# baycom/tfrec

Measured on AMD Instinct MI355X. Metric: IQ MSamples/s through demod+decode (batched streams), higher is better.
Workload: dtype int32+f32+f64

## Files before the change

tfrec_amd/csrc/decode.h:

```cpp
#pragma once

__device__ __forceinline__ const uint32_t *win_bits(const WinTables &T, int c, int j, int og)
{
	return T.bits + (size_t)c * T.bit_words + (og >> 6) + 3 * j;
}

__device__ __forceinline__ uint32_t tfa1_sr_before(const WinTables &T, const ChainState &st, int c, int j)
{
	uint32_t sr = 0;
	int have = 0;
	for (int k = j - 1; k >= 0 && have < 32; k--) {
		const int nb = T.result[(size_t)c * T.cap + k].nbits;
		if (nb <= 0)
			continue;
		const uint32_t *bits = win_bits(T, c, k, T.open[(size_t)c * T.cap + k]);
		const int take = nb < 32 - have ? nb : 32 - have;
		const int p0 = nb - take;
		const uint32_t lo = bits[p0 >> 5], hi = ((p0 + take - 1) >> 5) != (p0 >> 5) ? bits[(p0 >> 5) + 1] : 0u;
		const unsigned long long w = ((unsigned long long)hi << 32) | lo;
		const uint32_t piece = (uint32_t)(w >> (p0 & 31)) & (take >= 32 ? ~0u : (1u << take) - 1u);
		sr = (have == 0) ? (take >= 32 ? piece : piece << (32 - take))
				 : (sr | (piece << (32 - have - take)));
		have += take;
	}
	if (have < 32)
		sr |= have ? (st.sr >> have) : st.sr;
	return sr;
}

template <int KIND>
__device__ __forceinline__ void decode_window(int c, int j, int n_streams, const ChainLaunch &L, const WinTables &T,
					      uint8_t *__restrict__ my_rdata)
{
	const int a = c / n_streams, s = c - a * n_streams;
	const ChainState &st = L.states[a][s];
	const WinResult r = T.result[(size_t)c * T.cap + j];
	const int og = T.open[(size_t)c * T.cap + j];
	const uint32_t *bits = win_bits(T, c, j, og);
	Dec d{ 0u, -1, 0, 0, 0, 0, 0, 0, 0, 0u, 0u, my_rdata };
	if (j == 0) {
		const uint4 *src = reinterpret_cast<const uint4 *>(st.rdata);
		uint4 *dst = reinterpret_cast<uint4 *>(my_rdata);
#pragma unroll
		for (int q = 0; q < 4; q++)
			dst[q] = src[q];
		d.sr = st.sr;
		d.sr_cnt = st.sr_cnt;
		d.byte_cnt = st.byte_cnt;
		d.invert = st.invert;
	} else if (KIND == 0) {
		d.sr = tfa1_sr_before(T, st, c, j);
	}
	int maxlen = d.byte_cnt;
	const int nbits = r.nbits;
	uint32_t wnext = nbits > 0 ? bits[0] : 0u;
	for (int n = 0; n < nbits; n += 32) {
		const uint32_t wbits = wnext;
		if (n + 32 < nbits)
			wnext = bits[(n >> 5) + 1];
		const int cnt = nbits - n < 32 ? nbits - n : 32;
		for (int q = 0; q < cnt; q++) {
			store_bit<KIND>(d, (wbits >> q) & 1);
			maxlen = d.byte_cnt > maxlen ? d.byte_cnt : maxlen;
		}
	}
	WinDecode &o = T.decode[(size_t)c * T.cap + j];
	o.sr = d.sr;
	o.sr_cnt = d.sr_cnt;
	o.byte_cnt = d.byte_cnt;
	o.invert = d.invert;
	o.wlen = j == 0 ? 64 : (maxlen < 64 ? maxlen : 64);
	const uint4 *src = reinterpret_cast<const uint4 *>(my_rdata);
	uint4 *dst = reinterpret_cast<uint4 *>(o.vals);
#pragma unroll
	for (int q = 0; q < 4; q++)
		dst[q] = src[q];
}

__global__ __launch_bounds__(64) void decode_kernel(int n_streams, ChainLaunch L, WinTables T, int kind)
{
	__builtin_amdgcn_s_setprio(3);
	__shared__ __attribute__((aligned(16))) uint8_t rdata_lds[64 * 256];
	uint8_t *my_rdata = rdata_lds + 256 * threadIdx.x;
	const size_t total = (size_t)L.n_active * n_streams * T.cap;
	const uint32_t tid = blockIdx.x * 64 + threadIdx.x, nthreads = gridDim.x * 64;
	for (int q = 2 * kind; q < 2 * kind + 2; q++) {
		const uint32_t count = T.queue[q].count;
		for (uint32_t idx = tid; idx < count; idx += nthreads) {
			const uint2 it = T.items[(size_t)q * total + idx];
			if (kind == 0)
				decode_window<0>((int)it.x, (int)it.y, n_streams, L, T, my_rdata);
			else
				decode_window<1>((int)it.x, (int)it.y, n_streams, L, T, my_rdata);
		}
	}
}

template <int KIND, bool WAVE>
__device__ __forceinline__ void commit_body(int a, int s, int n_streams, int n_blocks, long long sample_base,
					    const uint32_t *__restrict__ dec, size_t dec_stride,
					    const int16_t *__restrict__ ld16, const ChainLaunch &L, const WinTables &T,
					    tfrec_amd_event *__restrict__ events, EventBuf *__restrict__ eb, uint32_t flags,
					    uint8_t *__restrict__ my_rdata)
{
	const int M = n_blocks * kBlockDec;
	const ChainParams &p = L.params[a];
	ChainState &st = L.states[a][s];
	const int c = a * n_streams + s;
	const int count = T.count[c];
	const bool lead = !WAVE || threadIdx.x == 0;
	EmitCtx e{ events, eb, flags, (uint32_t)s, L.slot[a], p.sensor_type, sample_base, !lead };
	{
		const uint4 *src = reinterpret_cast<const uint4 *>(st.rdata);
		uint4 *dst = reinterpret_cast<uint4 *>(my_rdata);
#pragma unroll
		for (int q = 0; q < 4; q++)
			dst[q] = src[q];
	}
	Dec d{ st.sr, st.sr_cnt, st.byte_cnt, st.invert, st.synced, st.w_last_bit, st.psk, st.last_psk, st.nrzs, st.lfsr, st.seq,
	       my_rdata };
	if (KIND == 1 && !WAVE) {
		int lbi = st.last_bit_idx, lbi_block = -1;
		bool ok = true;
		for (int j = 0; j < count && ok; j++) {
			const int close = T.close[(size_t)c * T.cap + j];
			const int last = close < M ? close : M - 1;
			const WinResult *rr = &T.result[(size_t)c * T.cap + j];
			if (j > 0 && rr->first_cand_g >= 0) {
				const int index_c = 2 * (rr->first_cand_g & (kBlockDec - 1));
				const int lbi_c = rebase_lbi(lbi, lbi_block, rr->first_cand_g >> 13);
				const int tdiff = index_c - lbi_c;
				ok = (index_c > lbi_c + 8) && !(tdiff > p.spb / 4 && tdiff < 32 * p.spb);
			}
			lbi = (j == 0 || rr->first_cand_g >= 0) ? rr->lbi_out : rebase_lbi(lbi, lbi_block, last >> 13);
			lbi_block = last >> 13;
		}
		if (!ok) {
			const size_t total = (size_t)L.n_active * n_streams * T.cap;
			const uint32_t idx = atomicAdd(&T.queue[kDeferQueue].count, 1u);
			T.items[(size_t)kNQueues * total + idx] = make_uint2((uint32_t)a, (uint32_t)s);
			return;
		}
	}
	int lbi = st.last_bit_idx;
	int lbi_block = -1;
	const WinResult *last_r = nullptr;
	for (int j = 0; j < count; j++) {
		const int og = T.open[(size_t)c * T.cap + j];
		const int close = T.close[(size_t)c * T.cap + j];
		const int last = close < M ? close : M - 1;
		WinResult *rr = &T.result[(size_t)c * T.cap + j];
		if (KIND == 1) {
			if (j > 0) {
				if (rr->first_cand_g >= 0) {
					const int bc = rr->first_cand_g >> 13;
					const int index_c = 2 * (rr->first_cand_g & (kBlockDec - 1));
					const int lbi_c = rebase_lbi(lbi, lbi_block, bc);
					const int tdiff = index_c - lbi_c;
					const bool same = (index_c > lbi_c + 8) && !(tdiff > p.spb / 4 && tdiff < 32 * p.spb);
					if (WAVE && !same) {
						if (lead)
							atomicAdd(&T.stats[3], 1ull);
						GroupStats unused = { 0, 0 };
						coop_tfa2(c, j, n_streams, M, dec, dec_stride, ld16, L, T, nullptr, unused, true,
							  rebase_lbi(lbi, lbi_block, og >> 13));
						__threadfence();
						__syncthreads();
						uint4 keep[4];
#pragma unroll
						for (int q = 0; q < 4; q++)
							keep[q] = reinterpret_cast<uint4 *>(my_rdata)[q];
						decode_window<1>(c, j, n_streams, L, T, my_rdata);
#pragma unroll
						for (int q = 0; q < 4; q++)
							reinterpret_cast<uint4 *>(my_rdata)[q] = keep[q];
					}
					lbi = rr->lbi_out;
				} else {
					lbi = rebase_lbi(lbi, lbi_block, last >> 13);
				}
			} else {
				lbi = rr->lbi_out;
			}
			lbi_block = last >> 13;
		}
		const WinDecode *wd = &T.decode[(size_t)c * T.cap + j];
		const int wl = wd->wlen;
		const uint32_t *vsrc = reinterpret_cast<const uint32_t *>(wd->vals);
		uint32_t *vdst = reinterpret_cast<uint32_t *>(my_rdata);
		for (int b = 0; b < wl; b += 4) {
			const uint32_t v = vsrc[b >> 2];
			if (wl - b >= 4)
				vdst[b >> 2] = v;
			else {
				const uint32_t m = (1u << (8 * (wl - b))) - 1u;
				vdst[b >> 2] = (vdst[b >> 2] & ~m) | (v & m);
			}
		}
		d.sr = wd->sr;
		d.sr_cnt = wd->sr_cnt;
		d.byte_cnt = wd->byte_cnt;
		d.invert = wd->invert;
		if ((flags & TFREC_AMD_F_BITS) && rr->nbits > 0)
			emit_bits(e, d.seq, og, 0, win_bits(T, c, j, og), rr->nbits);
		if (rr->closed)
			flush<KIND>(e, d, rr->rssi_i, KIND == 1 ? rr->offset : 0, last);
		last_r = rr;
	}
	if (!lead)
		return;
	const bool open_at_end = last_r && !last_r->closed;
	if (open_at_end) {
		st.mark_lvl = last_r->mark_lvl;
		st.rssi_i = last_r->rssi_i;
		st.bitcnt = last_r->bitcnt;
		st.dmin = last_r->dmin;
		st.dmax = last_r->dmax;
		st.offset = last_r->offset;
		st.last_bit = last_r->last_bit;
	} else {
		st.mark_lvl = 0;
		st.rssi_i = 0;
		st.bitcnt = 0;
		st.dmin = 32767;
		st.dmax = -32767;
		st.offset = 0;
		st.last_bit = 0;
	}
	if (KIND == 0)
		st.last_bit_idx = open_at_end ? rebase_lbi(last_r->lbi_out, (M - 1) >> 13, n_blocks - 1) : 0;
	else
		st.last_bit_idx = rebase_lbi(lbi, lbi_block, n_blocks - 1);
	st.timeout_cnt = T.timeout_next[c];
	{
		const uint32_t lw = dec[(size_t)s * dec_stride + M - 1];
		st.prev_i = (int)(int16_t)(lw & 0xffff);
		st.prev_q = (int)lw >> 16;
	}
	{
		const uint4 *src = reinterpret_cast<const uint4 *>(my_rdata);
		uint4 *dst = reinterpret_cast<uint4 *>(st.rdata);
#pragma unroll
		for (int q = 0; q < 4; q++)
			dst[q] = src[q];
	}
	st.sr = d.sr;
	st.sr_cnt = d.sr_cnt;
	st.byte_cnt = d.byte_cnt;
	st.invert = d.invert;
	st.synced = d.synced;
	st.seq = d.seq;
}

__global__ __launch_bounds__(64) void commit_kernel(const uint32_t *__restrict__ dec, size_t dec_stride,
						    const int16_t *__restrict__ ld16, int n_streams, int n_blocks,
						    long long sample_base, ChainLaunch L, WinTables T,
						    tfrec_amd_event *__restrict__ events, EventBuf *__restrict__ eb, uint32_t flags,
						    int lanes, int want_kind)
{
	__builtin_amdgcn_s_setprio(3);
	__shared__ __attribute__((aligned(16))) uint8_t rdata_lds[64 * 256];
	uint8_t *my_rdata = rdata_lds + 256 * threadIdx.x;
	const int a = blockIdx.y;
	const int s = blockIdx.x * lanes + threadIdx.x;
	if ((int)threadIdx.x >= lanes || s >= n_streams)
		return;
	const int kind = L.params[a].kind;
	if (kind != want_kind)
		return;
	if (kind == 0)
		commit_body<0, false>(a, s, n_streams, n_blocks, sample_base, dec, dec_stride, ld16, L, T, events, eb, flags, my_rdata);
	else if (kind == 1)
		commit_body<1, false>(a, s, n_streams, n_blocks, sample_base, dec, dec_stride, ld16, L, T, events, eb, flags, my_rdata);
}

__global__ __launch_bounds__(64) void commit_wave_kernel(const uint32_t *__restrict__ dec, size_t dec_stride,
							 const int16_t *__restrict__ ld16, int n_streams, int n_blocks,
							 long long sample_base, ChainLaunch L, WinTables T,
							 tfrec_amd_event *__restrict__ events, EventBuf *__restrict__ eb,
							 uint32_t flags)
{
	__builtin_amdgcn_s_setprio(3);
	__shared__ __attribute__((aligned(16))) uint8_t rdata_lds[256];
	const size_t total = (size_t)L.n_active * n_streams * T.cap;
	const uint32_t count = T.queue[kDeferQueue].count;
	for (uint32_t idx = blockIdx.x; idx < count; idx += gridDim.x) {
		const uint2 it = T.items[(size_t)kNQueues * total + idx];
		commit_body<1, true>((int)it.x, (int)it.y, n_streams, n_blocks, sample_base, dec, dec_stride, ld16, L, T, events, eb,
				     flags, rdata_lds);
		__syncthreads();
	}
}
```

tfrec_amd/csrc/whb_check.h:

```cpp
#pragma once

#ifndef TFREC_AMD_CHK_STREAMS
#define TFREC_AMD_CHK_STREAMS 32
#endif
constexpr int kChkStreams = TFREC_AMD_CHK_STREAMS;
constexpr int kChkProducers = 2;
constexpr int kChkPerProducer = kChkStreams / kChkProducers;
static_assert(kChkStreams <= 64 && kChkStreams % kChkProducers == 0, "a lane per stream, the streams split evenly");
constexpr int kChkPairRow = 64 * 4 + 4;
constexpr int kChkDevRow = 64 + 4;
struct ChkBuf {
	uint32_t pair[kChkStreams * kChkPairRow];
	uint32_t dev[kChkStreams * kChkDevRow];
};
constexpr size_t kChkLdsBytes = 2 * sizeof(ChkBuf);

__global__ __launch_bounds__(64 * (1 + kChkProducers)) void whb_chain_kernel(int n_streams, ChainLaunch L, int a, WinTables T)
{
	extern __shared__ __attribute__((aligned(16))) uint8_t chk_lds[];
	ChkBuf *const buf = reinterpret_cast<ChkBuf *>(chk_lds);
	const int wave = (int)threadIdx.x >> 6, ln = (int)threadIdx.x & 63;
	const int s0 = (int)blockIdx.x * kChkStreams;
	const ChainParams &p = L.params[a];
	const double a1 = p.iir_avg.a1, a2 = p.iir_avg.a2, bh = 0.5 * p.iir_avg.b0;
	const int my_s = s0 + ln;
	const bool my_on = ln < kChkStreams && my_s < n_streams;
	const int my_rounds = my_on ? T.whbdense_n[my_s] >> 6 : 0;
	int rmax = my_rounds;
#pragma unroll
	for (int o = 32; o >= 1; o >>= 1) {
		const int other = __shfl_xor(rmax, o, 64);
		rmax = other > rmax ? other : rmax;
	}
	rmax = __builtin_amdgcn_readfirstlane(rmax);
	if (rmax == 0)
		return;
	if (wave == 0) {
		double y1 = 0.0, y2 = 0.0;
		if (my_on) {
			const WhbExact st = T.whbx[my_s];
			y1 = st.y1;
			y2 = st.y2;
		}
		unsigned long long *const xbits = T.whbxbits + (size_t)(my_on ? my_s : 0) * T.whbx_stride;
		double2 *const xsnap = T.whbxsnap + (size_t)(my_on ? my_s : 0) * T.whbx_stride;
		__syncthreads();
		for (int r = 0; r < rmax; r++) {
			if (r < my_rounds) {
				const ChkBuf &b = buf[r & 1];
				const double2 *prow = reinterpret_cast<const double2 *>(b.pair + ln * kChkPairRow);
				const uint4 *drow = reinterpret_cast<const uint4 *>(b.dev + ln * kChkDevRow);
				uint32_t acc[2] = { 0u, 0u };
				double2 pq[2][8];
				uint4 dq[2][2];
				auto fetch = [&](int h, int g8) {
#pragma unroll
					for (int j = 0; j < 8; j++)
						pq[h][j] = prow[8 * g8 + j];
					dq[h][0] = drow[2 * g8];
					dq[h][1] = drow[2 * g8 + 1];
				};
				fetch(0, 0);
#pragma unroll
				for (int g8 = 0; g8 < 8; g8++) {
					const int h = g8 & 1;
					if (g8 + 1 < 8)
						fetch(h ^ 1, g8 + 1);
					const int dv[8] = { (int)dq[h][0].x, (int)dq[h][0].y, (int)dq[h][0].z, (int)dq[h][0].w,
							    (int)dq[h][1].x, (int)dq[h][1].y, (int)dq[h][1].z, (int)dq[h][1].w };
#pragma unroll
					for (int j = 0; j < 8; j++) {
						const double P = pq[h][j].x, B2 = pq[h][j].y;
						const double y = ((B2 + a1 * y1) + P) + a2 * y2;
						y2 = y1;
						y1 = y;
						const int yi = (int)y;
						asm("v_cmp_lt_i32 vcc, %1, %2\n\tv_addc_co_u32 %0, vcc, %0, %0, vcc" : "+v"(acc[g8 >> 2]) : "v"(dv[j]), "v"(yi) : "vcc");
					}
				}
				xbits[r] = (unsigned long long)__brev(acc[0]) | ((unsigned long long)__brev(acc[1]) << 32);
				xsnap[r] = make_double2(y1, y2);
			}
			__syncthreads();
		}
	} else {
		const int q0 = (wave - 1) * kChkPerProducer;
		int rounds[kChkPerProducer], h1[kChkPerProducer], h2[kChkPerProducer];
		const int32_t *row[kChkPerProducer];
#pragma unroll
		for (int q = 0; q < kChkPerProducer; q++) {
			const int s = s0 + q0 + q;
			const bool on = s < n_streams;
			rounds[q] = __builtin_amdgcn_readlane(my_rounds, (q0 + q) & 63);
			row[q] = T.whbdense + (size_t)(on ? s : 0) * T.whbdense_stride;
			const WhbExact st = T.whbx[on ? s : 0];
			h1[q] = __builtin_amdgcn_readfirstlane(st.fd1);
			h2[q] = __builtin_amdgcn_readfirstlane(st.fd2);
		}
		int cur[kChkPerProducer], nxt[kChkPerProducer];
#pragma unroll
		for (int q = 0; q < kChkPerProducer; q++) {
			cur[q] = rounds[q] > 0 ? row[q][ln] : 0;
			nxt[q] = rounds[q] > 1 ? row[q][64 + ln] : 0;
		}
		auto lay_out = [&](ChkBuf &b, int r) {
#pragma unroll
			for (int q = 0; q < kChkPerProducer; q++) {
				if (r < rounds[q]) {
					const int d0 = cur[q];
					const int s1 = __builtin_amdgcn_update_dpp(0, d0, 0x138, 0xf, 0xf, false);
					const int d1 = ln == 0 ? h1[q] : s1;
					const int s2 = __builtin_amdgcn_update_dpp(0, d1, 0x138, 0xf, 0xf, false);
					const int d2 = ln == 0 ? h2[q] : s2;
					const double t0 = bh * (double)d0, t1 = bh * (double)d1, t2 = bh * (double)d2;
					const double P = __builtin_fma(2.0, t1, t0);
					*reinterpret_cast<double2 *>(b.pair + (q0 + q) * kChkPairRow + 4 * ln) = make_double2(P, t2);
					b.dev[(q0 + q) * kChkDevRow + ln] = (uint32_t)d0;
					h1[q] = __builtin_amdgcn_readlane(d0, 63);
					h2[q] = __builtin_amdgcn_readlane(d0, 62);
				}
			}
		};
		lay_out(buf[0], 0);
		__syncthreads();
		for (int r = 0; r < rmax; r++) {
			int far[kChkPerProducer];
#pragma unroll
			for (int q = 0; q < kChkPerProducer; q++)
				far[q] = r + 2 < rounds[q] ? row[q][64 * (r + 2) + ln] : 0;
#pragma unroll
			for (int q = 0; q < kChkPerProducer; q++)
				cur[q] = nxt[q];
			if (r + 1 < rmax)
				lay_out(buf[(r + 1) & 1], r + 1);
#pragma unroll
			for (int q = 0; q < kChkPerProducer; q++)
				nxt[q] = far[q];
			__syncthreads();
		}
	}
}

constexpr int kChkLockCap = 256;
__global__ __launch_bounds__(64) void whb_check_kernel(int n_streams, ChainLaunch L, int a, WinTables T, int *__restrict__ carry_io)
{
	__shared__ int lk_pos[kChkLockCap], lk_avgf[kChkLockCap];
	__shared__ uint32_t lk_meta[kChkLockCap];
	const int s = (int)blockIdx.x, ln = (int)threadIdx.x;
	if (s >= n_streams)
		return;
	const ChainParams &p = L.params[a];
	const double a1 = p.iir_avg.a1, a2 = p.iir_avg.a2, bh = 0.5 * p.iir_avg.b0;
	const int N = T.whbdense_n[s], R = N >> 6;
	const int32_t *dense = T.whbdense + (size_t)s * T.whbdense_stride;
	const unsigned long long *xbits = T.whbxbits + (size_t)s * T.whbx_stride;
	const double2 *xsnap = T.whbxsnap + (size_t)s * T.whbx_stride;
	const WhbExact st0 = T.whbx[s];
	const int tp_ = whb_hook_perturb(T);
	const int tol = tp_ > 1 ? tp_ : (tp_ < -1 ? -tp_ : 1);
	auto input = [&](int pos) -> int { return pos >= 0 ? dense[pos] : (pos == -1 ? st0.fd1 : st0.fd2); };
	auto run = [&](int rr, int cnt, double &y1, double &y2, unsigned long long &bits) {
		const int p0 = 64 * rr;
		if (rr == 0) {
			y1 = st0.y1;
			y2 = st0.y2;
		} else {
			const double2 sn = xsnap[rr - 1];
			y1 = sn.x;
			y2 = sn.y;
		}
		double t1 = bh * (double)input(p0 - 1), t2 = bh * (double)input(p0 - 2);
		bits = 0ull;
		for (int k = 0; k < cnt; k++) {
			const int d = dense[p0 + k];
			const double t0 = bh * (double)d;
			const double P = __builtin_fma(2.0, t1, t0);
			const double y = ((t2 + a1 * y1) + P) + a2 * y2;
			bits |= (unsigned long long)(d < (int)y ? 1u : 0u) << k;
			y2 = y1;
			y1 = y;
			t2 = t1;
			t1 = t0;
		}
	};
	double yf1 = 0.0, yf2 = 0.0;
	unsigned long long tailbits = 0ull;
	if (ln == 0)
		run(R, N & 63, yf1, yf2, tailbits);
	tailbits = __shfl(tailbits, 0, 64);
	auto word = [&](int i) -> unsigned long long { return i < R ? xbits[i] : (i == R ? tailbits : 0ull); };
	const uint4 *recrow = reinterpret_cast<const uint4 *>(T.whbrec + (size_t)s * T.whbrec_stride);
	int carry = carry_io[s];
	const int carry_in = carry;
	bool bad = false;
	int cbase = 0, nlocks = 0;
	bool ended = false;
	int last_delta = 0;
	bool have_last = false, last_closed = false;
	auto do_locks = [&]() {
		for (int b0 = 0; b0 < nlocks; b0 += 64) {
			const int i = b0 + ln;
			const bool on = i < nlocks;
			double y1 = 0.0, y2 = 0.0;
			unsigned long long bits;
			const int pos = on ? lk_pos[i] : 0;
			run(pos >> 6, on ? (pos & 63) + 1 : 0, y1, y2, bits);
			const uint32_t meta = on ? lk_meta[i] : 0u;
			const int delta = (int)y1 - (on ? lk_avgf[i] : 0);
			const bool b = on && (delta > tol || delta < -tol || (delta != 0 && (meta & kWhbRecAmb)));
			bad = bad || __ballot(b) != 0ull;
			const int nb = nlocks - b0 < 64 ? nlocks - b0 : 64;
			last_delta = __shfl(delta, nb - 1, 64);
			last_closed = (__shfl((int)meta, nb - 1, 64) & (int)kWhbRecClosed) != 0;
			have_last = true;
		}
		nlocks = 0;
	};
	for (int v0 = 0; !ended; v0 += 64) {
		const int vi = v0 + ln < T.whbrec_stride - 1 ? v0 + ln : T.whbrec_stride - 1;
		const uint4 rec = recrow[vi];
		const uint32_t meta = rec.z;
		const unsigned long long endm = __ballot(meta == kWhbRecEnd);
		const int nrec = endm ? __builtin_ctzll(endm) : 64;
		ended = endm != 0ull || v0 + 64 + 64 > T.whbrec_stride;
		const bool on = ln < nrec;
		const bool pseudo = on && (meta & kWhbRecPseudo) != 0u;
		const bool normal = on && !pseudo;
		const int nv = normal ? (int)((meta >> kWhbRecNvShift) & 63u) + 1 : 0;
		int inc = nv;
#pragma unroll
		for (int o = 1; o < 64; o <<= 1) {
			const int up = __shfl_up(inc, o, 64);
			inc += ln >= o ? up : 0;
		}
		const int pos0 = cbase + inc - nv;
		cbase += __shfl(inc, 63, 64);
		if (pseudo) {
			if (v0 + ln == 0) {
				bad = bad || (carry != 0 && (meta & kWhbRecAmb));
				if (meta & kWhbRecClosed)
					carry = 0;
			} else {
				bad = true;
			}
		}
		if (normal) {
			const int w = pos0 >> 6, sh = pos0 & 63;
			const unsigned long long lo = word(w) >> sh, hi = sh ? word(w + 1) << (64 - sh) : 0ull;
			const unsigned long long vm = nv >= 64 ? ~0ull : (1ull << nv) - 1ull;
			const unsigned long long below = ((unsigned long long)rec.y << 32) | rec.x;
			bad = bad || (((lo | hi) ^ below) & vm) != 0ull || pos0 + nv > N;
		}
		carry = __shfl(carry, 0, 64);
		const bool lock = normal && (meta & kWhbRecLock) != 0u;
		const unsigned long long lm = __ballot(lock);
		if (lm) {
			if (nlocks + 64 > kChkLockCap)
				do_locks();
			if (lock) {
				const int i = nlocks + __builtin_popcountll(lm & ((1ull << ln) - 1ull));
				lk_pos[i] = pos0 + nv - 1;
				lk_avgf[i] = (int)rec.w;
				lk_meta[i] = meta;
			}
			nlocks += __builtin_popcountll(lm);
			__syncthreads();
		}
	}
	if (nlocks)
		do_locks();
	bad = __ballot(bad) != 0ull || cbase != N;
	if (have_last)
		carry = last_closed ? 0 : last_delta;
	if (ln == 0) {
		WhbExact st = st0;
		st.carry = carry_in;
		st.pad_ = 0;
		T.whbx0[s] = st;
		bad = bad || T.whbseen[s] != T.whbgen[s];
		if (whb_hook_force_fail(T) > 0 && (s + T.whb_submit_seq) % whb_hook_force_fail(T) == 0)
			bad = true;
		st.y1 = yf1;
		st.y2 = yf2;
		st.fd1 = input(N - 1);
		st.fd2 = input(N - 2);
		st.carry = st.pad_ = 0;
		T.whbx[s] = st;
		carry_io[s] = bad ? 0 : carry;
		T.whbfail[s] = bad ? 1 : 0;
	}
}
```

Baseline: 299,300.

## Prefetch window records in commit and group record loads in WHB check

The commit loop now loads each window's result and decode fields into registers one window ahead, so global-memory latency for window j+1 overlaps the work on window j. The defer precheck batches its loads in groups of 8. The WHB check kernel fetches records several 64-wide groups ahead, preloads the dense input for the IIR replay as uint4 vectors, and restructures when lock batches are flushed. In exchange it uses more registers, which may lower occupancy, and the group and flush logic is more complex and easier to get wrong.

```diff
diff --git a/tfrec_amd/csrc/decode.h b/tfrec_amd/csrc/decode.h
--- a/tfrec_amd/csrc/decode.h
+++ b/tfrec_amd/csrc/decode.h
@@ -96,6 +96,18 @@
 	}
 }
 
+#ifndef TFREC_AMD_COMMIT_AHEAD
+#define TFREC_AMD_COMMIT_AHEAD 1
+#endif
+constexpr int kCommitAhead = TFREC_AMD_COMMIT_AHEAD;
+struct CommitWin {
+	int og, close;
+	int nbits, closed, rssi_i, offset, lbi_out, first_cand_g;
+	uint32_t sr;
+	int sr_cnt, byte_cnt, invert, wlen;
+	uint4 vals[4];
+};
+
 template <int KIND, bool WAVE>
 __device__ __forceinline__ void commit_body(int a, int s, int n_streams, int n_blocks, long long sample_base,
 					    const uint32_t *__restrict__ dec, size_t dec_stride,
@@ -122,18 +134,32 @@
 	if (KIND == 1 && !WAVE) {
 		int lbi = st.last_bit_idx, lbi_block = -1;
 		bool ok = true;
-		for (int j = 0; j < count && ok; j++) {
-			const int close = T.close[(size_t)c * T.cap + j];
-			const int last = close < M ? close : M - 1;
-			const WinResult *rr = &T.result[(size_t)c * T.cap + j];
-			if (j > 0 && rr->first_cand_g >= 0) {
-				const int index_c = 2 * (rr->first_cand_g & (kBlockDec - 1));
-				const int lbi_c = rebase_lbi(lbi, lbi_block, rr->first_cand_g >> 13);
-				const int tdiff = index_c - lbi_c;
-				ok = (index_c > lbi_c + 8) && !(tdiff > p.spb / 4 && tdiff < 32 * p.spb);
-			}
-			lbi = (j == 0 || rr->first_cand_g >= 0) ? rr->lbi_out : rebase_lbi(lbi, lbi_block, last >> 13);
-			lbi_block = last >> 13;
+		constexpr int kPreGroup = 8;
+		for (int j0 = 0; j0 < count && ok; j0 += kPreGroup) {
+			int close_g[kPreGroup], cand_g[kPreGroup], lbi_g[kPreGroup];
+#pragma unroll
+			for (int g = 0; g < kPreGroup; g++) {
+				const size_t i = (size_t)c * T.cap + (j0 + g < count ? j0 + g : count - 1);
+				close_g[g] = T.close[i];
+				cand_g[g] = T.result[i].first_cand_g;
+				lbi_g[g] = T.result[i].lbi_out;
+			}
+#pragma unroll
+			for (int g = 0; g < kPreGroup; g++) {
+				const int j = j0 + g;
+				if (j < count && ok) {
+					const int close = close_g[g], first_cand_g = cand_g[g];
+					const int last = close < M ? close : M - 1;
+					if (j > 0 && first_cand_g >= 0) {
+						const int index_c = 2 * (first_cand_g & (kBlockDec - 1));
+						const int lbi_c = rebase_lbi(lbi, lbi_block, first_cand_g >> 13);
+						const int tdiff = index_c - lbi_c;
+						ok = (index_c > lbi_c + 8) && !(tdiff > p.spb / 4 && tdiff < 32 * p.spb);
+					}
+					lbi = (j == 0 || first_cand_g >= 0) ? lbi_g[g] : rebase_lbi(lbi, lbi_block, last >> 13);
+					lbi_block = last >> 13;
+				}
+			}
 		}
 		if (!ok) {
 			const size_t total = (size_t)L.n_active * n_streams * T.cap;
@@ -145,16 +171,41 @@
 	int lbi = st.last_bit_idx;
 	int lbi_block = -1;
 	const WinResult *last_r = nullptr;
-	for (int j = 0; j < count; j++) {
-		const int og = T.open[(size_t)c * T.cap + j];
-		const int close = T.close[(size_t)c * T.cap + j];
-		const int last = close < M ? close : M - 1;
+	constexpr int kSets = kCommitAhead + 1;
+	CommitWin w[kSets];
+	auto load_win = [&](int j, CommitWin &o) {
+		const size_t i = (size_t)c * T.cap + (j < count ? j : count - 1);
+		o.og = T.open[i];
+		o.close = T.close[i];
+		const WinResult *rr = &T.result[i];
+		o.nbits = rr->nbits;
+		o.closed = rr->closed;
+		o.rssi_i = rr->rssi_i;
+		if (KIND == 1) {
+			o.offset = rr->offset;
+			o.lbi_out = rr->lbi_out;
+			o.first_cand_g = rr->first_cand_g;
+		}
+		const WinDecode *wd = &T.decode[i];
+		o.sr = wd->sr;
+		o.sr_cnt = wd->sr_cnt;
+		o.byte_cnt = wd->byte_cnt;
+		o.invert = wd->invert;
+		o.wlen = wd->wlen;
+		const uint4 *vsrc = reinterpret_cast<const uint4 *>(wd->vals);
+#pragma unroll
+		for (int q = 0; q < 4; q++)
+			o.vals[q] = vsrc[q];
+	};
+	auto window = [&](int j, CommitWin &cw) {
+		const int og = cw.og;
+		const int last = cw.close < M ? cw.close : M - 1;
 		WinResult *rr = &T.result[(size_t)c * T.cap + j];
 		if (KIND == 1) {
 			if (j > 0) {
-				if (rr->first_cand_g >= 0) {
-					const int bc = rr->first_cand_g >> 13;
-					const int index_c = 2 * (rr->first_cand_g & (kBlockDec - 1));
+				if (cw.first_cand_g >= 0) {
+					const int bc = cw.first_cand_g >> 13;
+					const int index_c = 2 * (cw.first_cand_g & (kBlockDec - 1));
 					const int lbi_c = rebase_lbi(lbi, lbi_block, bc);
 					const int tdiff = index_c - lbi_c;
 					const bool same = (index_c > lbi_c + 8) && !(tdiff > p.spb / 4 && tdiff < 32 * p.spb);
@@ -174,38 +225,54 @@
 #pragma unroll
 						for (int q = 0; q < 4; q++)
 							reinterpret_cast<uint4 *>(my_rdata)[q] = keep[q];
+						load_win(j, cw);
 					}
-					lbi = rr->lbi_out;
+					lbi = cw.lbi_out;
 				} else {
 					lbi = rebase_lbi(lbi, lbi_block, last >> 13);
 				}
 			} else {
-				lbi = rr->lbi_out;
+				lbi = cw.lbi_out;
 			}
 			lbi_block = last >> 13;
 		}
-		const WinDecode *wd = &T.decode[(size_t)c * T.cap + j];
-		const int wl = wd->wlen;
-		const uint32_t *vsrc = reinterpret_cast<const uint32_t *>(wd->vals);
+		const int wl = cw.wlen;
 		uint32_t *vdst = reinterpret_cast<uint32_t *>(my_rdata);
-		for (int b = 0; b < wl; b += 4) {
-			const uint32_t v = vsrc[b >> 2];
+#pragma unroll
+		for (int b = 0; b < 64; b += 4) {
+			const uint4 v4 = cw.vals[b >> 4];
+			const uint32_t v = ((b >> 2) & 3) == 0 ? v4.x : (((b >> 2) & 3) == 1 ? v4.y : (((b >> 2) & 3) == 2 ? v4.z : v4.w));
 			if (wl - b >= 4)
 				vdst[b >> 2] = v;
-			else {
+			else if (wl - b > 0) {
 				const uint32_t m = (1u << (8 * (wl - b))) - 1u;
 				vdst[b >> 2] = (vdst[b >> 2] & ~m) | (v & m);
 			}
 		}
-		d.sr = wd->sr;
-		d.sr_cnt = wd->sr_cnt;
-		d.byte_cnt = wd->byte_cnt;
-		d.invert = wd->invert;
-		if ((flags & TFREC_AMD_F_BITS) && rr->nbits > 0)
-			emit_bits(e, d.seq, og, 0, win_bits(T, c, j, og), rr->nbits);
-		if (rr->closed)
-			flush<KIND>(e, d, rr->rssi_i, KIND == 1 ? rr->offset : 0, last);
+		d.sr = cw.sr;
+		d.sr_cnt = cw.sr_cnt;
+		d.byte_cnt = cw.byte_cnt;
+		d.invert = cw.invert;
+		if ((flags & TFREC_AMD_F_BITS) && cw.nbits > 0)
+			emit_bits(e, d.seq, og, 0, win_bits(T, c, j, og), cw.nbits);
+		if (cw.closed)
+			flush<KIND>(e, d, cw.rssi_i, KIND == 1 ? cw.offset : 0, last);
 		last_r = rr;
+	};
+	if (count > 0) {
+#pragma unroll
+		for (int r = 0; r < kCommitAhead; r++)
+			load_win(r, w[r]);
+		for (int j0 = 0; j0 < count; j0 += kSets) {
+#pragma unroll
+			for (int r = 0; r < kSets; r++) {
+				const int j = j0 + r;
+				if (j >= count)
+					break;
+				load_win(j + kCommitAhead, w[(r + kCommitAhead) % kSets]);
+				window(j, w[r]);
+			}
+		}
 	}
 	if (!lead)
 		return;
diff --git a/tfrec_amd/csrc/whb_check.h b/tfrec_amd/csrc/whb_check.h
--- a/tfrec_amd/csrc/whb_check.h
+++ b/tfrec_amd/csrc/whb_check.h
@@ -142,6 +142,15 @@
 }
 
 constexpr int kChkLockCap = 256;
+#ifndef TFREC_AMD_CHK_GROUP
+#define TFREC_AMD_CHK_GROUP 4
+#endif
+constexpr int kChkGroup = TFREC_AMD_CHK_GROUP;
+struct ChkRound {
+	uint4 q[16];
+	int dm1, dm2;
+	double2 sn;
+};
 __global__ __launch_bounds__(64) void whb_check_kernel(int n_streams, ChainLaunch L, int a, WinTables T, int *__restrict__ carry_io)
 {
 	__shared__ int lk_pos[kChkLockCap], lk_avgf[kChkLockCap];
@@ -159,37 +168,63 @@
 	const int tp_ = whb_hook_perturb(T);
 	const int tol = tp_ > 1 ? tp_ : (tp_ < -1 ? -tp_ : 1);
 	auto input = [&](int pos) -> int { return pos >= 0 ? dense[pos] : (pos == -1 ? st0.fd1 : st0.fd2); };
-	auto run = [&](int rr, int cnt, double &y1, double &y2, unsigned long long &bits) {
+	auto fetch = [&](int rr, ChkRound &in) {
 		const int p0 = 64 * rr;
-		if (rr == 0) {
-			y1 = st0.y1;
-			y2 = st0.y2;
-		} else {
-			const double2 sn = xsnap[rr - 1];
-			y1 = sn.x;
-			y2 = sn.y;
-		}
-		double t1 = bh * (double)input(p0 - 1), t2 = bh * (double)input(p0 - 2);
+		const uint4 *src = reinterpret_cast<const uint4 *>(dense + p0);
+#pragma unroll
+		for (int g = 0; g < 16; g++)
+			in.q[g] = src[g];
+		in.dm1 = dense[rr ? p0 - 1 : 0];
+		in.dm2 = dense[rr ? p0 - 2 : 0];
+		in.sn = xsnap[rr ? rr - 1 : 0];
+	};
+	auto run = [&](int rr, int cnt, const ChkRound &in, double &y1, double &y2, unsigned long long &bits) {
+		y1 = rr ? in.sn.x : st0.y1;
+		y2 = rr ? in.sn.y : st0.y2;
+		double t1 = bh * (double)(rr ? in.dm1 : st0.fd1), t2 = bh * (double)(rr ? in.dm2 : st0.fd2);
 		bits = 0ull;
-		for (int k = 0; k < cnt; k++) {
-			const int d = dense[p0 + k];
-			const double t0 = bh * (double)d;
-			const double P = __builtin_fma(2.0, t1, t0);
-			const double y = ((t2 + a1 * y1) + P) + a2 * y2;
-			bits |= (unsigned long long)(d < (int)y ? 1u : 0u) << k;
-			y2 = y1;
-			y1 = y;
-			t2 = t1;
-			t1 = t0;
+#pragma unroll
+		for (int g = 0; g < 16; g++) {
+			if (__ballot(4 * g < cnt) == 0ull)
+				break;
+			const int dv[4] = { (int)in.q[g].x, (int)in.q[g].y, (int)in.q[g].z, (int)in.q[g].w };
+#pragma unroll
+			for (int j = 0; j < 4; j++) {
+				const int k = 4 * g + j;
+				if (k < cnt) {
+					const int d = dv[j];
+					const double t0 = bh * (double)d;
+					const double P = __builtin_fma(2.0, t1, t0);
+					const double y = ((t2 + a1 * y1) + P) + a2 * y2;
+					bits |= (unsigned long long)(d < (int)y ? 1u : 0u) << k;
+					y2 = y1;
+					y1 = y;
+					t2 = t1;
+					t1 = t0;
+				}
+			}
 		}
 	};
+	const uint4 *recrow = reinterpret_cast<const uint4 *>(T.whbrec + (size_t)s * T.whbrec_stride);
+	uint4 rec[kChkGroup];
+	auto load_group = [&](int v) {
+#pragma unroll
+		for (int g = 0; g < kChkGroup; g++) {
+			const int vi = v + 64 * g + ln < T.whbrec_stride - 1 ? v + 64 * g + ln : T.whbrec_stride - 1;
+			rec[g] = recrow[vi];
+		}
+	};
+	load_group(0);
+	const int fdn1 = input(N - 1), fdn2 = input(N - 2);
 	double yf1 = 0.0, yf2 = 0.0;
 	unsigned long long tailbits = 0ull;
-	if (ln == 0)
-		run(R, N & 63, yf1, yf2, tailbits);
+	{
+		ChkRound in;
+		fetch(R, in);
+		run(R, ln == 0 ? N & 63 : 0, in, yf1, yf2, tailbits);
+	}
 	tailbits = __shfl(tailbits, 0, 64);
-	auto word = [&](int i) -> unsigned long long { return i < R ? xbits[i] : (i == R ? tailbits : 0ull); };
-	const uint4 *recrow = reinterpret_cast<const uint4 *>(T.whbrec + (size_t)s * T.whbrec_stride);
+	auto word = [&](int i, unsigned long long x) -> unsigned long long { return i < R ? x : (i == R ? tailbits : 0ull); };
 	int carry = carry_io[s];
 	const int carry_in = carry;
 	bool bad = false;
@@ -198,13 +233,17 @@
 	int last_delta = 0;
 	bool have_last = false, last_closed = false;
 	auto do_locks = [&]() {
+		__syncthreads();
 		for (int b0 = 0; b0 < nlocks; b0 += 64) {
 			const int i = b0 + ln;
 			const bool on = i < nlocks;
 			double y1 = 0.0, y2 = 0.0;
 			unsigned long long bits;
 			const int pos = on ? lk_pos[i] : 0;
-			run(pos >> 6, on ? (pos & 63) + 1 : 0, y1, y2, bits);
+			const int rr = pos >> 6 < R ? pos >> 6 : R;
+			ChkRound in;
+			fetch(rr, in);
+			run(rr, on ? (pos & 63) + 1 : 0, in, y1, y2, bits);
 			const uint32_t meta = on ? lk_meta[i] : 0u;
 			const int delta = (int)y1 - (on ? lk_avgf[i] : 0);
 			const bool b = on && (delta > tol || delta < -tol || (delta != 0 && (meta & kWhbRecAmb)));
@@ -216,59 +255,83 @@
 		}
 		nlocks = 0;
 	};
-	for (int v0 = 0; !ended; v0 += 64) {
-		const int vi = v0 + ln < T.whbrec_stride - 1 ? v0 + ln : T.whbrec_stride - 1;
-		const uint4 rec = recrow[vi];
-		const uint32_t meta = rec.z;
-		const unsigned long long endm = __ballot(meta == kWhbRecEnd);
-		const int nrec = endm ? __builtin_ctzll(endm) : 64;
-		ended = endm != 0ull || v0 + 64 + 64 > T.whbrec_stride;
-		const bool on = ln < nrec;
-		const bool pseudo = on && (meta & kWhbRecPseudo) != 0u;
-		const bool normal = on && !pseudo;
-		const int nv = normal ? (int)((meta >> kWhbRecNvShift) & 63u) + 1 : 0;
-		int inc = nv;
-#pragma unroll
-		for (int o = 1; o < 64; o <<= 1) {
-			const int up = __shfl_up(inc, o, 64);
-			inc += ln >= o ? up : 0;
-		}
-		const int pos0 = cbase + inc - nv;
-		cbase += __shfl(inc, 63, 64);
-		if (pseudo) {
-			if (v0 + ln == 0) {
-				bad = bad || (carry != 0 && (meta & kWhbRecAmb));
-				if (meta & kWhbRecClosed)
-					carry = 0;
-			} else {
-				bad = true;
-			}
-		}
-		if (normal) {
-			const int w = pos0 >> 6, sh = pos0 & 63;
-			const unsigned long long lo = word(w) >> sh, hi = sh ? word(w + 1) << (64 - sh) : 0ull;
-			const unsigned long long vm = nv >= 64 ? ~0ull : (1ull << nv) - 1ull;
-			const unsigned long long below = ((unsigned long long)rec.y << 32) | rec.x;
-			bad = bad || (((lo | hi) ^ below) & vm) != 0ull || pos0 + nv > N;
-		}
-		carry = __shfl(carry, 0, 64);
-		const bool lock = normal && (meta & kWhbRecLock) != 0u;
-		const unsigned long long lm = __ballot(lock);
-		if (lm) {
-			if (nlocks + 64 > kChkLockCap)
-				do_locks();
+	int v0 = 0;
+	for (;;) {
+		uint4 cur[kChkGroup];
+#pragma unroll
+		for (int g = 0; g < kChkGroup; g++)
+			cur[g] = rec[g];
+		load_group(v0 + 64 * kChkGroup);
+		bool full = false;
+		bool normal[kChkGroup];
+		int pos0[kChkGroup], nv[kChkGroup];
+		unsigned long long wlo[kChkGroup], whi[kChkGroup];
+#pragma unroll
+		for (int g = 0; g < kChkGroup; g++) {
+			const uint32_t meta = cur[g].z;
+			const unsigned long long endm = __ballot(meta == kWhbRecEnd);
+			const int left = T.whbrec_stride - v0;
+			int nrec = endm ? __builtin_ctzll(endm) : 64;
+			nrec = nrec < left ? nrec : left;
+			const bool is_lock = ln < nrec && (meta & (kWhbRecPseudo | kWhbRecLock)) == kWhbRecLock;
+			full = full || (!ended && __ballot(is_lock) != 0ull && nlocks + 64 > kChkLockCap);
+			const bool take = !full && !ended;
+			const bool on = take && ln < nrec;
+			const bool pseudo = on && (meta & kWhbRecPseudo) != 0u;
+			normal[g] = on && !pseudo;
+			const bool lock = normal[g] && (meta & kWhbRecLock) != 0u;
+			const unsigned long long lm = __ballot(lock);
+			ended = ended || (take && (endm != 0ull || v0 + 64 >= T.whbrec_stride));
+			nv[g] = normal[g] ? (int)((meta >> kWhbRecNvShift) & 63u) + 1 : 0;
+			int inc = nv[g];
+#pragma unroll
+			for (int o = 1; o < 64; o <<= 1) {
+				const int up = __shfl_up(inc, o, 64);
+				inc += ln >= o ? up : 0;
+			}
+			pos0[g] = cbase + inc - nv[g];
+			cbase += __shfl(inc, 63, 64);
+			if (pseudo) {
+				if (v0 + ln == 0) {
+					bad = bad || (carry != 0 && (meta & kWhbRecAmb));
+					if (meta & kWhbRecClosed)
+						carry = 0;
+				} else {
+					bad = true;
+				}
+			}
+			carry = __shfl(carry, 0, 64);
+			{
+				const int w = normal[g] ? pos0[g] >> 6 : 0;
+				wlo[g] = xbits[w < R ? w : 0];
+				whi[g] = xbits[w + 1 < R ? w + 1 : 0];
+			}
 			if (lock) {
 				const int i = nlocks + __builtin_popcountll(lm & ((1ull << ln) - 1ull));
-				lk_pos[i] = pos0 + nv - 1;
-				lk_avgf[i] = (int)rec.w;
+				lk_pos[i] = pos0[g] + nv[g] - 1;
+				lk_avgf[i] = (int)cur[g].w;
 				lk_meta[i] = meta;
 			}
 			nlocks += __builtin_popcountll(lm);
-			__syncthreads();
-		}
-	}
-	if (nlocks)
-		do_locks();
+			v0 += take ? 64 : 0;
+		}
+#pragma unroll
+		for (int g = 0; g < kChkGroup; g++) {
+			if (normal[g]) {
+				const int w = pos0[g] >> 6, sh = pos0[g] & 63;
+				const unsigned long long lo = word(w, wlo[g]) >> sh, hi = sh ? word(w + 1, whi[g]) << (64 - sh) : 0ull;
+				const unsigned long long vm = nv[g] >= 64 ? ~0ull : (1ull << nv[g]) - 1ull;
+				const unsigned long long below = ((unsigned long long)cur[g].y << 32) | cur[g].x;
+				bad = bad || (((lo | hi) ^ below) & vm) != 0ull || pos0[g] + nv[g] > N;
+			}
+		}
+		if (full || ended)
+			do_locks();
+		if (ended)
+			break;
+		if (full)
+			load_group(v0);
+	}
 	bad = __ballot(bad) != 0ull || cbase != N;
 	if (have_last)
 		carry = last_closed ? 0 : last_delta;
@@ -282,8 +345,8 @@
 			bad = true;
 		st.y1 = yf1;
 		st.y2 = yf2;
-		st.fd1 = input(N - 1);
-		st.fd2 = input(N - 2);
+		st.fd1 = fdn1;
+		st.fd2 = fdn2;
 		st.carry = st.pad_ = 0;
 		T.whbx[s] = st;
 		carry_io[s] = bad ? 0 : carry;
```

Result: no change. 301,500 (median of 6 runs) (+0.7%).
